# Patman86/SVT-AV1-Mod-by-Patman

Measured on AMD Instinct MI355X. Metric: encoded fps (4K 10-bit preset 8) + ME+txfm HBM GB/s vs roofline, 1/2/4/8 GPU, higher is better.
Workload: dtype u8 (ME) / int32 (transform)

## Files before the change

### include/svt_hip_txfm.h

```cpp
#ifndef SVT_HIP_TXFM_H
#define SVT_HIP_TXFM_H

#include "svt_hip.h"

#ifdef __cplusplus
extern "C" {
#endif

#define SVT_HIP_FWD_DECL(W, H)                                                                                     \
    SVT_HIP_API void svt_av1_fwd_txfm2d_##W##x##H##_hip(int16_t *input, int32_t *output, uint32_t input_stride,    \
                                                        int32_t transform_type, uint8_t bit_depth);               \
    SVT_HIP_API void svt_av1_fwd_txfm2d_##W##x##H##_N2_hip(int16_t *input, int32_t *output, uint32_t input_stride, \
                                                           int32_t transform_type, uint8_t bit_depth);            \
    SVT_HIP_API void svt_av1_fwd_txfm2d_##W##x##H##_N4_hip(int16_t *input, int32_t *output, uint32_t input_stride, \
                                                           int32_t transform_type, uint8_t bit_depth);
SVT_HIP_FWD_DECL(4, 4) SVT_HIP_FWD_DECL(8, 8) SVT_HIP_FWD_DECL(16, 16) SVT_HIP_FWD_DECL(32, 32) SVT_HIP_FWD_DECL(64, 64)
SVT_HIP_FWD_DECL(4, 8) SVT_HIP_FWD_DECL(8, 4) SVT_HIP_FWD_DECL(8, 16) SVT_HIP_FWD_DECL(16, 8) SVT_HIP_FWD_DECL(16, 32)
SVT_HIP_FWD_DECL(32, 16) SVT_HIP_FWD_DECL(32, 64) SVT_HIP_FWD_DECL(64, 32) SVT_HIP_FWD_DECL(4, 16) SVT_HIP_FWD_DECL(16, 4)
SVT_HIP_FWD_DECL(8, 32) SVT_HIP_FWD_DECL(32, 8) SVT_HIP_FWD_DECL(16, 64) SVT_HIP_FWD_DECL(64, 16)

SVT_HIP_API uint64_t svt_handle_transform16x64_hip(int32_t *output);
SVT_HIP_API uint64_t svt_handle_transform32x64_hip(int32_t *output);
SVT_HIP_API uint64_t svt_handle_transform64x16_hip(int32_t *output);
SVT_HIP_API uint64_t svt_handle_transform64x32_hip(int32_t *output);
// ... 95 lines not shown
typedef struct SvtHipTxfmDesc {
    uint64_t residual_off;
    uint64_t coeff_off;
    uint64_t qcoeff_off, dqcoeff_off;
    uint64_t pred_off, recon_off;
    uint64_t iscan_off;
    uint64_t qm_off, iqm_off;
    uint32_t residual_stride;
    uint32_t pred_stride, recon_stride;
    int16_t  zbin[2], round[2], quant[2], quant_shift[2], dequant[2];
    uint8_t  tx_type, shape , bit_depth, quant_mode, log_scale, flags;
    uint8_t  dist_w, dist_h;
} SvtHipTxfmDesc;

typedef struct SvtHipTxfmResult {
    uint64_t three_quad_energy;
    uint16_t eob;
    uint16_t pad_;
    uint32_t satd;
} SvtHipTxfmResult;

SVT_HIP_API int32_t svt_hip_txfm_quant_batch(uint8_t *d_base, const SvtHipTxfmDesc *d_desc, SvtHipTxfmResult *d_result,
                                             uint32_t n_blocks, uint32_t w, uint32_t h, void *stream);

SVT_HIP_API int32_t svt_hip_txfm_distortion_batch(const uint8_t *d_base, const SvtHipTxfmDesc *d_desc, uint64_t (*d_distortion)[2],
                                                  uint32_t n_blocks, uint32_t w, uint32_t h, void *stream);

SVT_HIP_API int32_t svt_hip_quantize_batch(uint8_t *d_base, const SvtHipTxfmDesc *d_desc, SvtHipTxfmResult *d_result,
                                           uint32_t n_blocks, uint32_t n_coeffs, void *stream);

typedef struct SvtHipCoeffCost {
    int32_t txb_skip[13][2];
    int32_t base_eob[4][3];
    int32_t base[42][8];
    int32_t eob_extra[9][2];
    int32_t dc_sign[3][2];
    int32_t lps[21][26];
} SvtHipCoeffCost;

typedef struct SvtHipRateTables {
    SvtHipCoeffCost coeff[5][2];
    int32_t         eob[7][2][2][11];
    int32_t         intra_tx_type[3][4][13][17];
    int32_t         inter_tx_type[4][4][17];
} SvtHipRateTables;

// ... 164 lines not shown
```

### svt-av1-mod-by-patman_amd/csrc/common.hpp

```cpp
#pragma once

#include <hip/hip_runtime.h>
#include <stddef.h>
#include <stdint.h>
#include <string.h>

#include "../../include/svt_hip.h"
#include "../../include/svt_hip_me.h"

namespace svthip {

void set_error(const char *fmt, ...);

hipStream_t resolve_stream(void *stream);

struct Scratch {
    uint8_t *dev    = nullptr;
    uint8_t *pinned = nullptr;
    size_t   dev_cap = 0, pinned_cap = 0;
    uint8_t *device(size_t bytes);
    uint8_t *host(size_t bytes, size_t keep = 0);
};

bool ensure_init();
int  cu_count();
hipError_t ensure_event(hipEvent_t &ev);

struct GuardedBuf {
    uint8_t   *dev = nullptr, *pinned = nullptr;
    size_t     cap = 0;
    hipEvent_t ev  = nullptr;
    bool       pending = false;
    bool       held    = false;
    hipError_t acquire(size_t bytes, size_t grow_to, bool host_writes, hipStream_t st, const char **what);
    hipError_t release(hipStream_t st);
};

struct ThreadState {
    char       err[512] = "";
    bool       bound    = false;
    int        slot     = -1;
    GuardedBuf ring[4];
    int        ring_next = 0;
    Scratch    scratch;
    GuardedBuf wiener_aux;
    GuardedBuf txfm_perm;
    hipEvent_t produced = nullptr;
};
ThreadState &tls();

class TierBCall {
public:
    TierBCall(const char *fn, void *stream);
    ~TierBCall() { release(); }
    TierBCall(const TierBCall &)            = delete;
    TierBCall &operator=(const TierBCall &) = delete;
    bool        ok() const { return status_ == SVT_HIP_OK; }
    int32_t     status() const { return status_; }
    hipStream_t stream() const { return st_; }
    void       *stage(const void *host, size_t bytes);
    void       *take(GuardedBuf &b, size_t bytes, size_t grow_to);
    int32_t     finish();

private:
    void       *fail(hipError_t e, const char *what);
    bool        hold(GuardedBuf &b, size_t bytes, size_t grow_to, bool host_writes);
    void        release();
    const char *fn_;
    hipStream_t st_     = nullptr;
// ... 100 lines not shown
```

### svt-av1-mod-by-patman_amd/csrc/runtime.cpp

```cpp
#include <atomic>
#include <cstdarg>
#include <cstdio>
#include <cstdlib>
#include <cstring>
#include <mutex>

#include "common.hpp"

namespace svthip {

#ifndef SVT_HIP_STREAM_POOL
#define SVT_HIP_STREAM_POOL 8
#endif
namespace {
constexpr int STREAM_POOL = SVT_HIP_STREAM_POOL;
struct Process {
    std::atomic<int> device{-1};
    std::atomic<int> sticky{-1};
    std::atomic<int> cus{0};
    std::mutex       mutex;
    std::atomic<hipStream_t> pool[STREAM_POOL];
    std::mutex               pool_mutex;
    std::atomic<int>         next_thread{0};
};
// ... 122 lines not shown
}
bool TierBCall::hold(GuardedBuf &b, size_t bytes, size_t grow_to, bool host_writes) {
    if (!ok())
        return false;
    if (b.held)
        return fail(hipErrorInvalidValue, "buffer still held by an enclosing call") != nullptr;
    const char      *what;
    const hipError_t e = b.acquire(bytes, grow_to, host_writes, st_, &what);
    if (e != hipSuccess)
        return fail(e, what) != nullptr;
    b.held = true, held_[n_held_++] = &b;
    return true;
}
void *TierBCall::stage(const void *host, size_t bytes) {
    ThreadState &t = tls();
    GuardedBuf  &s = t.ring[t.ring_next];
    if (!hold(s, bytes, bytes < 65536 ? 65536 : bytes * 2, true))
        return nullptr;
    t.ring_next = (t.ring_next + 1) % 4;
    memcpy(s.pinned, host, bytes);
    const hipError_t e = hipMemcpyAsync(s.dev, s.pinned, bytes, hipMemcpyHostToDevice, st_);
    return e == hipSuccess ? s.dev : fail(e, "hipMemcpyAsync");
}
void *TierBCall::take(GuardedBuf &b, size_t bytes, size_t grow_to) { return hold(b, bytes, grow_to, false) ? b.dev : nullptr; }
void TierBCall::release() {
    for (int i = 0; i < n_held_; i++) {
        const hipError_t e = held_[i]->release(st_);
        if (e != hipSuccess)
            fail(e, "hipEventRecord");
        held_[i]->held = false;
    }
    n_held_ = 0;
}
int32_t TierBCall::finish() {
    const hipError_t e = ok() ? hipGetLastError() : hipSuccess;
    if (e != hipSuccess)
        fail(e, "launch");
    release();
    return status_;
}

namespace {
struct SavedSlot {
    char   name[96];
    void **slot;
    void  *cpu_fn;
};
// ... 352 lines not shown
```

### svt-av1-mod-by-patman_amd/csrc/txfm.hip

```cpp
#include <cmath>
#include <cstdio>
#include <cstdlib>
#include <cstring>
#include <mutex>

#include "../../include/svt_hip_txfm.h"
#include "common.hpp"
#include "txfm_block.hpp"

using namespace svthip;
using namespace svthip::txd;
using namespace svthip::txb;

namespace {

template <int W, int H>
__global__ __launch_bounds__((Geo<W, H>::NT * Geo<W, H>::L), (Geo<W, H>::MINW)) void txfm_kernel(uint8_t *__restrict__ base,
                                                                            const SvtHipTxfmDesc *__restrict__ descs,
                                                                            SvtHipTxfmResult *__restrict__ results,
                                                                            uint32_t n, const uint32_t *__restrict__ perm) {
    using G = Geo<W, H>;
    constexpr int L = G::L, PW = G::PW, NT = G::NT;
    __shared__ int32_t buf[NT][H * PW];
    const int          t = threadIdx.x % L, slot = threadIdx.x / L;
    const uint32_t     i    = blockIdx.x * NT + slot;
    const bool         live = i < n;
    const uint32_t     tb   = live ? (perm ? perm[i] : i) : 0;
    txfm_block<W, H>(base, descs[tb], results + tb, live, t, buf[slot]);
}

constexpr uint32_t GROUP_CHUNK = 4096, GROUP_MIN_BLOCKS = 2048;
__global__ __launch_bounds__(1024) void group_by_type_kernel(const SvtHipTxfmDesc *__restrict__ descs, uint32_t n, uint32_t *__restrict__ perm) {
    __shared__ uint32_t hist[16], start[16];
    const uint32_t base = blockIdx.x * GROUP_CHUNK;
    if (threadIdx.x < 16)
        hist[threadIdx.x] = 0;
    __syncthreads();
    uint32_t key[GROUP_CHUNK / 1024], rank[GROUP_CHUNK / 1024];
#pragma unroll
    for (uint32_t k = 0; k < GROUP_CHUNK / 1024; k++) {
        const uint32_t i = base + k * 1024 + threadIdx.x;
        key[k] = i < n ? (descs[i].tx_type & 15u) : 16u;
        if (key[k] < 16)
            rank[k] = atomicAdd(&hist[key[k]], 1u);
    }
    __syncthreads();
// ... 82 lines not shown
std::once_flag g_tables_once;
int32_t        g_tables_rc = SVT_HIP_OK;
void           upload_tables() {
    constexpr CosTable tab = make_cospi();
    for (int b = 0; b < 4; b++)
        for (int j = 0; j < 64; j++)
            if (tab.v[b][j] != (int32_t)llround(cos(M_PI * j / 128.0) * (double)(1 << (10 + b)))) {
                set_error("transform constant table self-check failed");
                g_tables_rc = SVT_HIP_ERR_RUNTIME;
            }
}
}

int32_t svthip::txfm_ready() {
    if (!ensure_init())
        return SVT_HIP_ERR_NO_DEVICE;
    std::call_once(g_tables_once, upload_tables);
    return g_tables_rc;
}

namespace {

template <int W, int H>
void launch_txfm(uint8_t *base, const SvtHipTxfmDesc *descs, SvtHipTxfmResult *res, uint32_t n, hipStream_t st) {
    using G = Geo<W, H>;
    const uint32_t *perm = nullptr;
    static const bool group = getenv("SVTAV1_HIP_GROUP_TX") != nullptr;
    if (G::NT > 1 && n >= GROUP_MIN_BLOCKS && group && st) {
        TierBCall c("transform grouping", (void *)st);
        perm = (const uint32_t *)c.take(tls().txfm_perm, (size_t)n * sizeof(uint32_t), (size_t)n * sizeof(uint32_t));
        if (perm)
            hipLaunchKernelGGL(group_by_type_kernel, dim3((n + GROUP_CHUNK - 1) / GROUP_CHUNK), dim3(1024), 0, st, descs, n, (uint32_t *)perm);
        hipLaunchKernelGGL((txfm_kernel<W, H>), dim3((n + G::NT - 1) / G::NT), dim3(G::NT * G::L), 0, st, base, descs, res, n, perm);
        return;
    }
    hipLaunchKernelGGL((txfm_kernel<W, H>), dim3((n + G::NT - 1) / G::NT), dim3(G::NT * G::L), 0, st, base, descs, res, n, perm);
}

bool dispatch_txfm(uint32_t w, uint32_t h, uint8_t *base, const SvtHipTxfmDesc *descs, SvtHipTxfmResult *res, uint32_t n,
                   hipStream_t st) {
#define CASE(W, H)                                \
    if (w == W && h == H) {                       \
        launch_txfm<W, H>(base, descs, res, n, st); \
        return true;                              \
    }
    CASE(4, 4) CASE(8, 8) CASE(16, 16) CASE(32, 32) CASE(64, 64) CASE(4, 8) CASE(8, 4) CASE(8, 16) CASE(16, 8) CASE(16, 32)
    CASE(32, 16) CASE(32, 64) CASE(64, 32) CASE(4, 16) CASE(16, 4) CASE(8, 32) CASE(32, 8) CASE(16, 64) CASE(64, 16)
#undef CASE
    return false;
}

}

extern "C" int32_t svt_hip_txfm_quant_batch(uint8_t *d_base, const SvtHipTxfmDesc *d_desc, SvtHipTxfmResult *d_result,
                                            uint32_t n_blocks, uint32_t w, uint32_t h, void *stream) {
    if (!d_base || !d_desc || !d_result) {
        set_error("svt_hip_txfm_quant_batch: NULL pointer");
        return SVT_HIP_ERR_BAD_PARAMETER;
    }
    const int32_t rc = txfm_ready();
    if (rc != SVT_HIP_OK)
        return rc;
    if (n_blocks == 0)
        return SVT_HIP_OK;
    if (!dispatch_txfm(w, h, d_base, d_desc, d_result, n_blocks, resolve_stream(stream))) {
        set_error("svt_hip_txfm_quant_batch: %ux%u is not an AV1 transform size", w, h);
        return SVT_HIP_ERR_BAD_PARAMETER;
    }
    SVT_HIP_CHECK(hipGetLastError());
    return SVT_HIP_OK;
}

extern "C" int32_t svt_hip_quantize_batch(uint8_t *d_base, const SvtHipTxfmDesc *d_desc, SvtHipTxfmResult *d_result,
                                          uint32_t n_blocks, uint32_t n_coeffs, void *stream) {
    if (!d_base || !d_desc || !d_result || n_coeffs == 0) {
        set_error("svt_hip_quantize_batch: bad argument");
        return SVT_HIP_ERR_BAD_PARAMETER;
    }
    const int32_t rc = txfm_ready();
    if (rc != SVT_HIP_OK)
        return rc;
    if (n_blocks == 0)
        return SVT_HIP_OK;
    hipLaunchKernelGGL(quantize_kernel, dim3(n_blocks), dim3(256), 0, resolve_stream(stream), d_base, d_desc, d_result, n_coeffs);
    SVT_HIP_CHECK(hipGetLastError());
    return SVT_HIP_OK;
}

namespace {


struct OneBlock : TierAStage {
    size_t off_desc, off_res;
    OneBlock(const char *what) : TierAStage(what, txfm_ready() == SVT_HIP_OK), off_desc(in(nullptr, 256)), off_res(out(256)) {
        memset(desc(), 0, sizeof(SvtHipTxfmDesc));
    }
    SvtHipTxfmDesc         *desc() const { return host<SvtHipTxfmDesc>(off_desc); }
    const SvtHipTxfmResult *result() const { return host<SvtHipTxfmResult>(off_res); }
    void run(int w, int h) {
        upload();
        if (!dispatch_txfm((uint32_t)w, (uint32_t)h, dev(0), dev<const SvtHipTxfmDesc>(off_desc), dev<SvtHipTxfmResult>(off_res), 1, stream()))
            fatal("bad transform size");
    }
};

void fwd_tier_a(int w, int h, int shape, int16_t *input, int32_t *output, uint32_t stride, int32_t tx_type, uint8_t bd) {
    OneBlock     a("forward transform");
    const size_t out_bytes = (size_t)w * h * 4;
    const size_t off_in = a.in(input, ((size_t)(h - 1) * stride + w) * 2, 16), off_out = a.out(out_bytes + 16);
    SvtHipTxfmDesc *dsc = a.desc();
    dsc->residual_off = off_in, dsc->coeff_off = off_out;
    dsc->qcoeff_off = dsc->dqcoeff_off = dsc->qm_off = dsc->iqm_off = dsc->iscan_off = dsc->pred_off = dsc->recon_off = SVT_HIP_NO_OFFSET;
    dsc->residual_stride = stride;
    dsc->tx_type = (uint8_t)tx_type, dsc->shape = (uint8_t)shape, dsc->bit_depth = bd;
    dsc->quant_mode = SVT_HIP_QUANT_NONE, dsc->flags = SVT_HIP_TX_FWD | SVT_HIP_TX_FULLCOEFF;
    a.run(w, h);
    a.finish(off_out, out_bytes);
    memcpy(output, a.host(off_out), out_bytes);
}

template <class PIX>
void inv_tier_a(int w, int h, const int32_t *input, const PIX *out_r, int32_t stride_r, PIX *out_w, int32_t stride_w, int32_t tx_type,
                int32_t bd) {
    OneBlock     a("inverse transform");
// ... 113 lines not shown
```

### svt-av1-mod-by-patman_amd/csrc/txfm_block.hpp

```cpp
#pragma once
#include <cstdint>

#include "../../include/svt_hip_txfm.h"
#include "common.hpp"
#include "txfm_device.hpp"

namespace svthip {
int32_t txfm_ready();
namespace txb {
using namespace svthip::txd;


constexpr int8_t FWD_SHIFT[5][5][3] = {
    {{2, 0, 0}, {2, -1, 0}, {2, -1, 0}, {0, 0, 0}, {0, 0, 0}},   {{2, -1, 0}, {2, -1, 0}, {2, -2, 0}, {2, -2, 0}, {0, 0, 0}},
    {{2, -1, 0}, {2, -2, 0}, {2, -2, 0}, {2, -4, 0}, {0, -2, 0}}, {{0, 0, 0}, {2, -2, 0}, {2, -4, 0}, {2, -4, 0}, {0, -2, -2}},
    {{0, 0, 0}, {0, 0, 0}, {2, -4, 0}, {2, -4, -2}, {0, -2, -2}}};
constexpr int8_t FWD_COS_COL[5][5] = {{13, 13, 13, 0, 0}, {13, 13, 13, 12, 0}, {13, 13, 13, 12, 13}, {0, 13, 13, 12, 13}, {0, 0, 13, 12, 13}};
constexpr int8_t FWD_COS_ROW[5][5] = {{13, 13, 12, 0, 0}, {13, 13, 13, 12, 0}, {13, 13, 12, 13, 12}, {0, 12, 13, 12, 11}, {0, 0, 12, 11, 10}};
constexpr int8_t INV_SHIFT0[5][5]  = {{0, 0, -1, 0, 0}, {0, -1, -1, -2, 0}, {-1, -1, -2, -1, -2}, {0, -2, -1, -2, -1}, {0, 0, -2, -1, -2}};
__device__ const uint8_t VTX_D[16] = {0, 1, 0, 1, 2, 0, 2, 1, 2, 3, 0, 3, 1, 3, 2, 3};
__device__ const uint8_t HTX_D[16] = {0, 0, 1, 1, 0, 2, 2, 2, 1, 3, 3, 0, 3, 1, 3, 2};

constexpr int cmax(int a, int b) { return a > b ? a : b; }
constexpr int cmin(int a, int b) { return a < b ? a : b; }
constexpr int pow2floor(int v) {
    int p = 1;
    while (p * 2 <= v) p *= 2;
    return p;
}
#ifndef SVT_HIP_TX64_WAVES
#define SVT_HIP_TX64_WAVES 1
#endif
template <int W, int H>
struct Geo {
    static constexpr int L  = cmax(W, H);
    static constexpr int PW = W + 1;
    static constexpr int NT = cmax(1, 64 / L);
    static constexpr int IW = cmin(W, 32), IH = cmin(H, 32);
    static constexpr int MINW = L == 32 ? 3 : (L == 8 ? 8 : (L == 64 ? SVT_HIP_TX64_WAVES : 1));
    static constexpr int WI = clog2(W) - 2, HI = clog2(H) - 2;
    static constexpr bool RECT = (W == 2 * H) || (H == 2 * W);
};

struct QP {
    int32_t        zbin[2], round[2], quant[2], qshift[2], dequant[2];
    int32_t        log_scale, mode;
    const uint8_t *qm, *iqm;
    bool           simple;
};
__device__ __forceinline__ int32_t rpot(int32_t v, int n) { return (v + ((1 << n) >> 1)) >> n; }
__device__ __forceinline__ void load_qp(QP &q, const SvtHipTxfmDesc &d, const uint8_t *base) {
    q.log_scale = d.log_scale, q.mode = d.quant_mode;
    bool small = true;
    for (int i = 0; i < 2; i++) {
        q.zbin[i]    = rpot(d.zbin[i], d.log_scale);
        q.round[i]   = rpot(d.round[i], d.log_scale);
        q.quant[i]   = d.quant[i];
        q.qshift[i]  = d.quant_shift[i];
        q.dequant[i] = d.dequant[i];
        small = small && q.zbin[i] >= 0 && q.zbin[i] < 65536 && q.round[i] >= 0 && q.round[i] < 32768 && q.quant[i] >= -32768 && q.quant[i] < 32768 &&
            q.qshift[i] >= 0 && q.qshift[i] < 65536 && q.dequant[i] >= 0 && q.dequant[i] < 32768;
    }
// ... 130 lines not shown
};

template <int IW, int IH, int L, int PW>
__device__ __forceinline__ void coop_store_tile(const int32_t *__restrict__ lds, int32_t *__restrict__ g, int t) {
    constexpr int NCH = IW * IH / 4;
    if ((((uintptr_t)g) & 15) == 0) {
#pragma unroll
        for (int k = 0; k < (NCH + L - 1) / L; k++) {
            const int q = k * L + t;
            if (q < NCH) {
                const int e = 4 * q, r = e / IW, c = e % IW;
                int4      v;
                v.x = lds[r * PW + c], v.y = lds[r * PW + c + 1], v.z = lds[r * PW + c + 2], v.w = lds[r * PW + c + 3];
                typedef int v4i __attribute__((ext_vector_type(4)));
                const v4i nv = {v.x, v.y, v.z, v.w};
                __builtin_nontemporal_store(nv, (v4i *)g + q);
            }
        }
    } else {
        for (int e = t; e < IW * IH; e += L) g[e] = lds[(e / IW) * PW + e % IW];
    }
}

template <int W, int H, bool BLKERR = false>
__device__ __forceinline__ void txfm_block(uint8_t *__restrict__ base, const SvtHipTxfmDesc &d, SvtHipTxfmResult *__restrict__ result,
                                           const bool live, const int t, int32_t *__restrict__ lds) {
    static_assert(!BLKERR || (W != 64 && H != 64), "three_quad_energy is the 64-point energy for those sizes");
    using G = Geo<W, H>;
    constexpr int L = G::L, PW = G::PW, IW = G::IW, IH = G::IH;
    const int vk = VTX_D[d.tx_type & 15], hk = HTX_D[d.tx_type & 15];
    const bool ud = vk == 2, lr = hk == 2;
    const int  bd = d.bit_depth;
    const int  bdi = bd == 8 ? 0 : (bd == 10 ? 1 : (bd == 12 ? 2 : -1));
    const bool do_fwd = d.flags & SVT_HIP_TX_FWD, do_inv = d.flags & SVT_HIP_TX_INV;
    constexpr int sh0 = FWD_SHIFT[G::WI][G::HI][0], sh1 = FWD_SHIFT[G::WI][G::HI][1], sh2 = FWD_SHIFT[G::WI][G::HI][2];
    int32_t  row[W];
#pragma unroll
    for (int c = 0; c < W; c++) row[c] = 0;

    if (do_fwd) {
        if (live && t < W) {
            int32_t        v[H];
            {
                const ptrdiff_t step = ud ? -(ptrdiff_t)d.residual_stride : (ptrdiff_t)d.residual_stride;
                const ptrdiff_t row0 = (ud ? (ptrdiff_t)(H - 1) * d.residual_stride : 0) + t;
                if (!(d.flags & SVT_HIP_TX_SRC_PRED)) {
                    const int16_t *rp = (const int16_t *)(base + d.residual_off) + row0;
#pragma unroll
                    for (int r = 0; r < H; r++, rp += step) v[r] = (int32_t)((uint32_t)(int32_t)__builtin_nontemporal_load(rp) << sh0);
                } else {
                    const ptrdiff_t pstep = ud ? -(ptrdiff_t)d.pred_stride : (ptrdiff_t)d.pred_stride;
                    const ptrdiff_t prow0 = (ud ? (ptrdiff_t)(H - 1) * d.pred_stride : 0) + t;
                    if (d.flags & SVT_HIP_TX_PIXEL16) {
                        const uint16_t *sp = (const uint16_t *)(base + d.residual_off) + row0;
                        const uint16_t *pp = (const uint16_t *)(base + d.pred_off) + prow0;
#pragma unroll
                        for (int r = 0; r < H; r++, sp += step, pp += pstep)
                            v[r] = (int32_t)((uint32_t)(int32_t)(int16_t)(*sp - *pp) << sh0);
                    } else {
                        const uint8_t *sp = base + d.residual_off + row0, *pp = base + d.pred_off + prow0;
#pragma unroll
                        for (int r = 0; r < H; r++, sp += step, pp += pstep) v[r] = (int32_t)((uint32_t)((int32_t)*sp - (int32_t)*pp) << sh0);
                    }
                }
            }
            if (__all(max_abs<H>(v) <= (uint32_t)FWD_FAST_LIMIT[G::HI][kind_index(vk)][FWD_COS_COL[G::WI][G::HI] - 10])) {
                fwd1d<Fast, H>(v, vk, FWD_COS_COL[G::WI][G::HI]);
                if constexpr (sh1 < 0) {
#pragma unroll
                    for (int r = 0; r < H; r++) v[r] = Fast::rs(v[r], -sh1);
                }
            } else {
                fwd1d<Exact, H>(v, vk, FWD_COS_COL[G::WI][G::HI]);
                if constexpr (sh1 < 0) {
#pragma unroll
                    for (int r = 0; r < H; r++) v[r] = rshift64(v[r], -sh1);
                }
            }
            const int cc = lr ? W - 1 - t : t;
#pragma unroll
            for (int r = 0; r < H; r++) lds[r * PW + cc] = v[r];
        }
        __syncthreads();
        if (live && t < H) {
#pragma unroll
            for (int c = 0; c < W; c++) row[c] = lds[t * PW + c];
            if (__all(max_abs<W>(row) <= (uint32_t)FWD_FAST_LIMIT[G::WI][kind_index(hk)][FWD_COS_ROW[G::WI][G::HI] - 10])) {
                fwd1d<Fast, W>(row, hk, FWD_COS_ROW[G::WI][G::HI]);
                if constexpr (sh2 < 0) {
#pragma unroll
                    for (int c = 0; c < W; c++) row[c] = Fast::rs(row[c], -sh2);
                }
            } else {
                fwd1d<Exact, W>(row, hk, FWD_COS_ROW[G::WI][G::HI]);
                if constexpr (sh2 < 0) {
#pragma unroll
                    for (int c = 0; c < W; c++) row[c] = rshift64(row[c], -sh2);
                }
            }
            const int kw = W >> d.shape, kh = H >> d.shape;
#pragma unroll
            for (int c = 0; c < W; c++) {
                int32_t x = row[c];
                if (G::RECT)
                    x = rshift64((int64_t)x * 5793, 12);
                row[c] = (t < kh && c < kw) ? x : 0;
            }
        }
    }
    uint64_t energy = 0;
    if constexpr (W == 64 || H == 64) {
        if (do_fwd && live && t < H) {
#pragma unroll
            for (int c = 0; c < W; c++)
                if (t >= IH || c >= IW)
                    energy += (uint64_t)((int64_t)row[c] * (int64_t)row[c]);
        }
        energy = group_sum64<L>(energy);
    }
    uint32_t satd = 0;
    if (do_fwd && (d.flags & SVT_HIP_TX_SATD)) {
        if (live && t < IH) {
#pragma unroll
            for (int c = 0; c < IW; c++) satd += (uint32_t)(row[c] < 0 ? -row[c] : row[c]);
        }
        satd = group_sum32<L>(satd);
    }
    uint32_t eob = 0;
    uint32_t iscv[(IW + 1) / 2];
    {
        const bool      qon = live && t < IH && d.quant_mode != SVT_HIP_QUANT_NONE;
        const uint16_t *isp = (const uint16_t *)(base + (qon ? d.iscan_off : 0)) + (qon ? t * IW : 0);
#pragma unroll
        for (int c = 0; c < IW; c += 2) iscv[c / 2] = qon ? ((uint32_t)isp[c] | ((uint32_t)isp[c + 1] << 16)) : 0u;
    }
    if (live && do_fwd && d.coeff_off != SVT_HIP_NO_OFFSET && (d.flags & SVT_HIP_TX_FULLCOEFF) && t < H) {
        int32_t *co = (int32_t *)(base + d.coeff_off) + t * W;
#pragma unroll
        for (int c = 0; c < W; c++) co[c] = row[c];
    }
    if (live && t < IH) {
        if (do_fwd && d.coeff_off != SVT_HIP_NO_OFFSET && !(d.flags & SVT_HIP_TX_FULLCOEFF)) {
            int32_t *co = (int32_t *)(base + d.coeff_off) + t * IW;
#pragma unroll
            for (int c = 0; c < IW; c++) co[c] = row[c];
        }
        if (d.quant_mode != SVT_HIP_QUANT_NONE) {
            QP q;
            load_qp(q, d, base);
            if (!do_fwd) {
                const int32_t *ci = (const int32_t *)(base + d.coeff_off) + t * IW;
#pragma unroll
                for (int c = 0; c < IW; c++) row[c] = ci[c];
            }
            const bool btype = q.mode == SVT_HIP_QUANT_B || q.mode == SVT_HIP_QUANT_B_HBD;
            const int  path  = (q.simple && max_abs<IW>(row) <= 32767u) ? (btype ? 1 : 2) : 0;
            const bool all1 = __all(path == 1), all2 = __all(path == 2);
#pragma unroll
            for (int c = 0; c < IW; c++) {
                const uint32_t rc = (uint32_t)(t * IW + c);
                const int      ac = (c > 0) | (t > 0);
                int32_t        qc, dqc;
                if (all1)
                    quant_small<true>(q, row[c], ac, qc, dqc);
                else if (all2)
                    quant_small<false>(q, row[c], ac, qc, dqc);
                else
                    quant_one(q, row[c], rc, qc, dqc);
                const uint32_t pos = qc ? ((iscv[c / 2] >> (16 * (c & 1))) & 0xffffu) + 1u : 0u;
                eob                = pos > eob ? pos : eob;
                lds[t * PW + c] = qc;
                if constexpr (BLKERR) {
                    const int64_t e = (int64_t)row[c] - (int64_t)dqc;
                    energy += (uint64_t)(e * e);
                }
                row[c]          = dqc;
            }
        } else if (do_inv && !do_fwd) {
            const int32_t *dqi = (const int32_t *)(base + d.dqcoeff_off) + t * IW;
#pragma unroll
            for (int c = 0; c < IW; c++) row[c] = dqi[c];
        }
    }
    eob = group_max<L>(eob);
    if constexpr (BLKERR)
        energy = group_sum64<L>(energy);
    {
        const bool quant = live && d.quant_mode != SVT_HIP_QUANT_NONE;
        __syncthreads();
        if (quant && d.qcoeff_off != SVT_HIP_NO_OFFSET)
            coop_store_tile<IW, IH, L, PW>(lds, (int32_t *)(base + d.qcoeff_off), t);
        __syncthreads();
        if (quant && t < IH) {
#pragma unroll
            for (int c = 0; c < IW; c++) lds[t * PW + c] = row[c];
        }
        __syncthreads();
        if (quant && d.dqcoeff_off != SVT_HIP_NO_OFFSET)
            coop_store_tile<IW, IH, L, PW>(lds, (int32_t *)(base + d.dqcoeff_off), t);
    }
    if (live && t == 0) {
        SvtHipTxfmResult r;
        r.three_quad_energy = energy;
        r.eob               = (uint16_t)eob;
        r.pad_ = 0, r.satd = satd;
        *result = r;
    }
    __syncthreads();
    if (live && do_inv && t < H) {
        const int range_row = bd == 8 ? 16 : (bd == 10 ? 18 : 20);
        const int clamp_in  = bd + 8;
        bool      any       = false;
#pragma unroll
        for (int c = 0; c < W; c++) {
            int32_t x = (t < IH && c < IW) ? row[c] : 0;
            if (G::RECT)
                x = rshift64((int64_t)x * 2896, 12);
            row[c] = clampv<true>(x, clamp_in);
            any |= row[c] != 0;
        }
        if (any) {
            constexpr int ish0 = INV_SHIFT0[G::WI][G::HI];
            if (__all(bdi >= 0 && INV_FAST_OK[bdi < 0 ? 0 : bdi][0][G::WI][kind_index(hk)] != 0)) {
                inv1d<Fast, W>(row, hk, range_row);
                if constexpr (ish0 < 0) {
#pragma unroll
                    for (int c = 0; c < W; c++) row[c] = Fast::rs(row[c], -ish0);
                }
            } else {
                inv1d<Exact, W>(row, hk, range_row);
                if constexpr (ish0 < 0) {
#pragma unroll
                    for (int c = 0; c < W; c++) row[c] = rshift64(row[c], -ish0);
                }
            }
        }
#pragma unroll
        for (int c = 0; c < W; c++) lds[t * PW + c] = row[c];
    }
    __syncthreads();
    if (live && do_inv && t < W) {
        int32_t   v[H];
        const int range_col = bd == 12 ? 18 : 16, col_clamp = bd + 6 > 16 ? bd + 6 : 16;
        const int cc = lr ? W - 1 - t : t;
#pragma unroll
        for (int r = 0; r < H; r++) v[r] = r < IH ? clampv<true>(lds[r * PW + cc], col_clamp) : 0;
        if (__all(bdi >= 0 && INV_FAST_OK[bdi < 0 ? 0 : bdi][1][G::HI][kind_index(vk)] != 0)) {
            inv1d<Fast, H>(v, vk, range_col);
#pragma unroll
            for (int r = 0; r < H; r++) v[r] = Fast::rs(v[r], 4);
        } else {
            inv1d<Exact, H>(v, vk, range_col);
#pragma unroll
            for (int r = 0; r < H; r++) v[r] = rshift64(v[r], 4);
        }
        const ptrdiff_t r0 = ud ? H - 1 : 0, rs = ud ? -(ptrdiff_t)d.recon_stride : (ptrdiff_t)d.recon_stride;
        uint32_t predv[(H + 1) / 2];
        {
            const ptrdiff_t ps = ud ? -(ptrdiff_t)d.pred_stride : (ptrdiff_t)d.pred_stride;
            if (d.flags & SVT_HIP_TX_PIXEL16) {
                const uint16_t *pr = (const uint16_t *)(base + d.pred_off) + r0 * (ptrdiff_t)d.pred_stride + t;
#pragma unroll
                for (int r = 0; r < H; r += 2) predv[r / 2] = (uint32_t)__builtin_nontemporal_load(pr + (ptrdiff_t)r * ps) | ((uint32_t)__builtin_nontemporal_load(pr + (ptrdiff_t)(r + 1) * ps) << 16);
            } else {
                const uint8_t *pr = base + d.pred_off + r0 * (ptrdiff_t)d.pred_stride + t;
#pragma unroll
                for (int r = 0; r < H; r += 2) predv[r / 2] = (uint32_t)pr[(ptrdiff_t)r * ps] | ((uint32_t)pr[(ptrdiff_t)(r + 1) * ps] << 16);
            }
        }
        const PixelClip clip((d.flags & SVT_HIP_TX_PIXEL16) ? bd : 8);
        if (d.flags & SVT_HIP_TX_PIXEL16) {
            uint16_t *rc = (uint16_t *)(base + d.recon_off) + r0 * (ptrdiff_t)d.recon_stride + t;
#pragma unroll
            for (int r = 0; r < H; r++, rc += rs) __builtin_nontemporal_store(clip.add((uint16_t)(predv[r / 2] >> (16 * (r & 1))), v[r]), rc);
        } else {
            uint8_t *rc = base + d.recon_off + r0 * (ptrdiff_t)d.recon_stride + t;
#pragma unroll
            for (int r = 0; r < H; r++, rc += rs) *rc = (uint8_t)clip.add((uint16_t)(predv[r / 2] >> (16 * (r & 1))), v[r]);
        }
    }
}

}
}
```

### svt-av1-mod-by-patman_amd/svtav1_hip/prototypes.py

```python
PROTOTYPES = {
    "svt_aom_cdef_find_dir_dual_hip": (None, ("c_void_p", "c_void_p", "c_int", "c_void_p", "c_void_p", "c_int32", "c_void_p", "c_void_p")),
    "svt_aom_cdef_find_dir_hip": ("c_uint8", ("c_void_p", "c_int32", "c_void_p", "c_int32")),
    "svt_aom_copy_rect8_8bit_to_16bit_hip": (None, ("c_void_p", "c_int32", "c_void_p", "c_int32", "c_int32", "c_int32")),
    "svt_aom_downsample_2d_hip": (None, ("c_void_p", "c_uint32", "c_uint32", "c_uint32", "c_void_p", "c_uint32", "c_uint32")),
    "svt_aom_highbd_lpf_horizontal_14_hip": (None, ("c_void_p", "c_int32", "c_void_p", "c_void_p", "c_void_p", "c_int32")),
    "svt_aom_highbd_lpf_horizontal_4_hip": (None, ("c_void_p", "c_int32", "c_void_p", "c_void_p", "c_void_p", "c_int32")),
    "svt_aom_highbd_lpf_horizontal_6_hip": (None, ("c_void_p", "c_int32", "c_void_p", "c_void_p", "c_void_p", "c_int32")),
    "svt_aom_highbd_lpf_horizontal_8_hip": (None, ("c_void_p", "c_int32", "c_void_p", "c_void_p", "c_void_p", "c_int32")),
    "svt_aom_highbd_lpf_vertical_14_hip": (None, ("c_void_p", "c_int32", "c_void_p", "c_void_p", "c_void_p", "c_int32")),
    "svt_aom_highbd_lpf_vertical_4_hip": (None, ("c_void_p", "c_int32", "c_void_p", "c_void_p", "c_void_p", "c_int32")),
    "svt_aom_highbd_lpf_vertical_6_hip": (None, ("c_void_p", "c_int32", "c_void_p", "c_void_p", "c_void_p", "c_int32")),
    "svt_aom_highbd_lpf_vertical_8_hip": (None, ("c_void_p", "c_int32", "c_void_p", "c_void_p", "c_void_p", "c_int32")),
    "svt_aom_highbd_quantize_b_hip": (None, ("c_void_p", "c_ssize_t", "c_void_p", "c_void_p", "c_void_p", "c_void_p", "c_void_p", "c_void_p", "c_void_p", "c_void_p", "c_void_p", "c_void_p", "c_void_p", "c_void_p", "c_int32")),
    "svt_aom_highbd_subtract_block_hip": (None, ("c_int", "c_int", "c_void_p", "c_ssize_t", "c_void_p", "c_ssize_t", "c_void_p", "c_ssize_t", "c_int")),
    "svt_aom_lpf_horizontal_14_hip": (None, ("c_void_p", "c_int32", "c_void_p", "c_void_p", "c_void_p")),
    "svt_aom_lpf_horizontal_4_hip": (None, ("c_void_p", "c_int32", "c_void_p", "c_void_p", "c_void_p")),
    "svt_aom_lpf_horizontal_6_hip": (None, ("c_void_p", "c_int32", "c_void_p", "c_void_p", "c_void_p")),
    "svt_aom_lpf_horizontal_8_hip": (None, ("c_void_p", "c_int32", "c_void_p", "c_void_p", "c_void_p")),
    "svt_aom_lpf_vertical_14_hip": (None, ("c_void_p", "c_int32", "c_void_p", "c_void_p", "c_void_p")),
    "svt_aom_lpf_vertical_4_hip": (None, ("c_void_p", "c_int32", "c_void_p", "c_void_p", "c_void_p")),
    "svt_aom_lpf_vertical_6_hip": (None, ("c_void_p", "c_int32", "c_void_p", "c_void_p", "c_void_p")),
    "svt_aom_lpf_vertical_8_hip": (None, ("c_void_p", "c_int32", "c_void_p", "c_void_p", "c_void_p")),
    "svt_aom_quantize_b_hip": (None, ("c_void_p", "c_ssize_t", "c_void_p", "c_void_p", "c_void_p", "c_void_p", "c_void_p", "c_void_p", "c_void_p", "c_void_p", "c_void_p", "c_void_p", "c_void_p", "c_void_p", "c_int32")),
    "svt_aom_sad_16b_kernel_hip": ("c_uint32", ("c_void_p", "c_uint32", "c_void_p", "c_uint32", "c_uint32", "c_uint32")),
# ... 133 lines not shown
    "svt_handle_transform64x16_hip": ("c_uint64", ("c_void_p",)),
    "svt_handle_transform64x32_N2_N4_hip": ("c_uint64", ("c_void_p",)),
    "svt_handle_transform64x32_hip": ("c_uint64", ("c_void_p",)),
    "svt_handle_transform64x64_N2_N4_hip": ("c_uint64", ("c_void_p",)),
    "svt_handle_transform64x64_hip": ("c_uint64", ("c_void_p",)),
    "svt_hip_analysis_frames": ("c_int32", ("c_void_p", "c_uint32", "c_int32", "c_int32", "c_void_p")),
    "svt_hip_blend_batch": ("c_int32", ("c_void_p", "c_uint32", "c_void_p")),
    "svt_hip_cdef_apply_frame": ("c_int32", ("c_void_p", "c_uint32", "c_void_p", "c_void_p", "c_int32", "c_int32", "c_void_p", "c_void_p", "c_void_p")),
    "svt_hip_cdef_apply_plane": ("c_int32", ("c_void_p", "c_void_p", "c_void_p", "c_int32", "c_int32", "c_void_p", "c_void_p", "c_void_p")),
    "svt_hip_cdef_pick_strengths": ("c_int32", ("c_void_p", "c_void_p", "c_void_p", "c_void_p", "c_void_p", "c_void_p", "c_void_p", "c_uint64", "c_void_p")),
    "svt_hip_cdef_pick_workspace_bytes": ("c_uint64", ("c_uint32", "c_int32")),
    "svt_hip_cdef_search_plane": ("c_int32", ("c_void_p", "c_void_p", "c_void_p", "c_void_p", "c_void_p", "c_void_p", "c_void_p")),
    "svt_hip_cfl_predict_batch": ("c_int32", ("c_void_p", "c_uint32", "c_void_p")),
    "svt_hip_comm_create": ("c_int32", ("c_void_p", "c_int32", "c_int32", "c_void_p")),
    "svt_hip_comm_destroy": ("c_int32", ("c_void_p",)),
    "svt_hip_comm_get_unique_id": ("c_int32", ("c_void_p",)),
    "svt_hip_compound_mask_search_batch": ("c_int32", ("c_void_p", "c_void_p", "c_uint32", "c_void_p")),
    "svt_hip_compute_units": ("c_int32", ()),
    "svt_hip_convolve_batch": ("c_int32", ("c_void_p", "c_uint32", "c_void_p")),
    "svt_hip_convolve_sr_batch": ("c_int32", ("c_void_p", "c_uint32", "c_void_p")),
    "svt_hip_copy": ("c_int32", ("c_void_p", "c_void_p", "c_size_t", "c_void_p")),
    "svt_hip_debug_inject_failure": (None, ("c_int32",)),
    "svt_hip_debug_tier_a_broken": ("c_int32", ("c_int32",)),
    "svt_hip_device_count": ("c_int32", ()),
    "svt_hip_download": ("c_int32", ("c_void_p", "c_void_p", "c_size_t", "c_void_p")),
    "svt_hip_download_2d": ("c_int32", ("c_void_p", "c_size_t", "c_void_p", "c_size_t", "c_size_t", "c_size_t", "c_void_p")),
    "svt_hip_event_destroy": ("c_int32", ("c_void_p",)),
    "svt_hip_free": ("c_int32", ("c_void_p",)),
    "svt_hip_gm_refine": ("c_int32", ("c_void_p", "c_void_p", "c_void_p", "c_int32", "c_int64", "c_void_p", "c_void_p")),
    "svt_hip_host_alloc": ("c_int32", ("c_void_p", "c_size_t")),
    "svt_hip_host_free": ("c_int32", ("c_void_p",)),
    "svt_hip_init": ("c_int32", ("c_int32",)),
    "svt_hip_install_rtcd": ("c_int32", ("c_void_p", "c_uint32", "c_void_p")),
    "svt_hip_install_rtcd_me": ("c_int32", ("c_void_p", "c_uint32")),
    "svt_hip_intra_predict_batch": ("c_int32", ("c_void_p", "c_uint32", "c_void_p")),
    "svt_hip_intra_predict_batch_packed": ("c_int32", ("c_void_p", "c_uint32", "c_uint32", "c_void_p")),
    "svt_hip_intra_search_frames": ("c_int32", ("c_void_p", "c_uint32", "c_void_p")),
    "svt_hip_last_error": ("c_char_p", ()),
    "svt_hip_loop_filter_frame": ("c_int32", ("c_void_p", "c_void_p")),
    "svt_hip_malloc": ("c_int32", ("c_void_p", "c_size_t")),
    "svt_hip_me_b64_count": ("c_uint32", ("c_uint32", "c_uint32")),
    "svt_hip_me_frames": ("c_int32", ("c_void_p", "c_uint32", "c_void_p")),
    "svt_hip_me_frames_dev": ("c_int32", ("c_void_p", "c_uint32", "c_uint32", "c_void_p")),
    "svt_hip_me_validate_jobs": ("c_int32", ("c_void_p", "c_uint32", "c_void_p")),
    "svt_hip_memset": ("c_int32", ("c_void_p", "c_int", "c_size_t", "c_void_p")),
    "svt_hip_pad_plane": ("c_int32", ("c_void_p", "c_void_p")),
# ... 65 lines not shown
```

Measured before the change: 5852.

## Add lean specialized transform kernel with device-side fallback list to general kernel

New measurement: 5980 (median of 6 runs). 1.02x the previous value.

```diff
diff --git a/include/svt_hip_txfm.h b/include/svt_hip_txfm.h
--- a/include/svt_hip_txfm.h
+++ b/include/svt_hip_txfm.h
@@ -141,6 +141,7 @@
 
 SVT_HIP_API int32_t svt_hip_txfm_quant_batch(uint8_t *d_base, const SvtHipTxfmDesc *d_desc, SvtHipTxfmResult *d_result,
                                              uint32_t n_blocks, uint32_t w, uint32_t h, void *stream);
+SVT_HIP_API int32_t svt_hip_debug_txfm_fallback_blocks(uint32_t *out);
 
 SVT_HIP_API int32_t svt_hip_txfm_distortion_batch(const uint8_t *d_base, const SvtHipTxfmDesc *d_desc, uint64_t (*d_distortion)[2],
                                                   uint32_t n_blocks, uint32_t w, uint32_t h, void *stream);
diff --git a/svt-av1-mod-by-patman_amd/csrc/common.hpp b/svt-av1-mod-by-patman_amd/csrc/common.hpp
--- a/svt-av1-mod-by-patman_amd/csrc/common.hpp
+++ b/svt-av1-mod-by-patman_amd/csrc/common.hpp
@@ -45,6 +45,8 @@
     Scratch    scratch;
     GuardedBuf wiener_aux;
     GuardedBuf txfm_perm;
+    hipStream_t     txfm_fast_stream = nullptr;
+    const uint32_t *txfm_fast_hdr    = nullptr;
     hipEvent_t produced = nullptr;
 };
 ThreadState &tls();
diff --git a/svt-av1-mod-by-patman_amd/csrc/runtime.cpp b/svt-av1-mod-by-patman_amd/csrc/runtime.cpp
--- a/svt-av1-mod-by-patman_amd/csrc/runtime.cpp
+++ b/svt-av1-mod-by-patman_amd/csrc/runtime.cpp
@@ -168,7 +168,12 @@
     const hipError_t e = hipMemcpyAsync(s.dev, s.pinned, bytes, hipMemcpyHostToDevice, st_);
     return e == hipSuccess ? s.dev : fail(e, "hipMemcpyAsync");
 }
-void *TierBCall::take(GuardedBuf &b, size_t bytes, size_t grow_to) { return hold(b, bytes, grow_to, false) ? b.dev : nullptr; }
+void *TierBCall::take(GuardedBuf &b, size_t bytes, size_t grow_to) {
+    ThreadState &t = tls();
+    if (&b == &t.txfm_perm)
+        t.txfm_fast_stream = nullptr, t.txfm_fast_hdr = nullptr;
+    return hold(b, bytes, grow_to, false) ? b.dev : nullptr;
+}
 void TierBCall::release() {
     for (int i = 0; i < n_held_; i++) {
         const hipError_t e = held_[i]->release(st_);
diff --git a/svt-av1-mod-by-patman_amd/csrc/txfm.hip b/svt-av1-mod-by-patman_amd/csrc/txfm.hip
--- a/svt-av1-mod-by-patman_amd/csrc/txfm.hip
+++ b/svt-av1-mod-by-patman_amd/csrc/txfm.hip
@@ -14,14 +14,51 @@
 
 namespace {
 
+enum : uint32_t { FB_COUNT = 0, FB_LIST = 16 };
+
 template <int W, int H>
-__global__ __launch_bounds__((Geo<W, H>::NT * Geo<W, H>::L), (Geo<W, H>::MINW)) void txfm_kernel(uint8_t *__restrict__ base,
+__global__ __launch_bounds__((Geo<W, H>::NT * Geo<W, H>::L), (Geo<W, H>::LEANW)) void txfm_kernel(uint8_t *__restrict__ base,
                                                                             const SvtHipTxfmDesc *__restrict__ descs,
                                                                             SvtHipTxfmResult *__restrict__ results,
-                                                                            uint32_t n, const uint32_t *__restrict__ perm) {
+                                                                            uint32_t n, const uint32_t *__restrict__ perm,
+                                                                            uint32_t *__restrict__ fb) {
+    using G = Geo<W, H>;
+    constexpr int L = G::L, PW = G::PW, NT = G::NT;
+    static_assert(NT * L == 64, "one wave per workgroup: a bail-out is uniform over the workgroup");
+    __shared__ int32_t buf[NT][H * PW];
+    const int          t = threadIdx.x % L, slot = threadIdx.x / L;
+    const uint32_t     i    = blockIdx.x * NT + slot;
+    const bool         live = i < n;
+    const uint32_t     tb   = live ? (perm ? perm[i] : i) : 0;
+    if constexpr (!G::LEAN) {
+        txfm_block<W, H>(base, descs[tb], results + tb, live, t, buf[slot]);
+    } else {
+        if (txfm_block<W, H, false, true>(base, descs[tb], results + tb, live, t, buf[slot]))
+            return;
+        const uint32_t left = n - blockIdx.x * NT, n_live = left < (uint32_t)NT ? left : (uint32_t)NT;
+        uint32_t       at   = 0;
+        if (threadIdx.x == 0)
+            at = atomicAdd(&fb[FB_COUNT], n_live);
+        at = (uint32_t)__shfl((int)at, 0, 64);
+        if (live && t == 0)
+            fb[FB_LIST + at + slot] = tb;
+    }
+}
+
+template <int W, int H>
+__global__ __launch_bounds__((Geo<W, H>::NT * Geo<W, H>::L), (Geo<W, H>::MINW)) void txfm_general_kernel(uint8_t *__restrict__ base,
+                                                                            const SvtHipTxfmDesc *__restrict__ descs,
+                                                                            SvtHipTxfmResult *__restrict__ results,
+                                                                            uint32_t n, const uint32_t *__restrict__ perm,
+                                                                            const uint32_t *__restrict__ count) {
     using G = Geo<W, H>;
     constexpr int L = G::L, PW = G::PW, NT = G::NT;
     __shared__ int32_t buf[NT][H * PW];
+    if (count) {
+        n = *count;
+        if (blockIdx.x * NT >= n)
+            return;
+    }
     const int          t = threadIdx.x % L, slot = threadIdx.x / L;
     const uint32_t     i    = blockIdx.x * NT + slot;
     const bool         live = i < n;
@@ -150,26 +187,48 @@
 namespace {
 
 template <int W, int H>
-void launch_txfm(uint8_t *base, const SvtHipTxfmDesc *descs, SvtHipTxfmResult *res, uint32_t n, hipStream_t st) {
+void launch_txfm(uint8_t *base, const SvtHipTxfmDesc *descs, SvtHipTxfmResult *res, uint32_t n, hipStream_t st, bool batch) {
     using G = Geo<W, H>;
     const uint32_t *perm = nullptr;
+    const dim3      grid((n + G::NT - 1) / G::NT), wg(G::NT * G::L);
+    ThreadState    &ts = tls();
+    auto            launch_general = [&](const uint32_t *pm) {
+        if constexpr (G::LEAN)
+            hipLaunchKernelGGL((txfm_general_kernel<W, H>), grid, wg, 0, st, base, descs, res, n, pm, (const uint32_t *)nullptr);
+        else
+            hipLaunchKernelGGL((txfm_kernel<W, H>), grid, wg, 0, st, base, descs, res, n, pm, (uint32_t *)nullptr);
+    };
+    ts.txfm_fast_stream = nullptr;
     static const bool group = getenv("SVTAV1_HIP_GROUP_TX") != nullptr;
-    if (G::NT > 1 && n >= GROUP_MIN_BLOCKS && group && st) {
-        TierBCall c("transform grouping", (void *)st);
-        perm = (const uint32_t *)c.take(tls().txfm_perm, (size_t)n * sizeof(uint32_t), (size_t)n * sizeof(uint32_t));
-        if (perm)
+    static const bool fast_on = !(getenv("SVTAV1_HIP_TXFM_FAST") && atoi(getenv("SVTAV1_HIP_TXFM_FAST")) == 0);
+    const bool fast = G::LEAN && fast_on && batch, grouped = G::NT > 1 && n >= GROUP_MIN_BLOCKS && group;
+    if ((fast || grouped) && st) {
+        TierBCall    c("transform scratch", (void *)st);
+        const size_t bytes = ((size_t)FB_LIST + (size_t)n * (grouped ? 2 : 1)) * sizeof(uint32_t);
+        uint32_t    *fb    = (uint32_t *)c.take(ts.txfm_perm, bytes, bytes);
+        if (fb && grouped) {
+            perm = fb + FB_LIST + n;
             hipLaunchKernelGGL(group_by_type_kernel, dim3((n + GROUP_CHUNK - 1) / GROUP_CHUNK), dim3(1024), 0, st, descs, n, (uint32_t *)perm);
-        hipLaunchKernelGGL((txfm_kernel<W, H>), dim3((n + G::NT - 1) / G::NT), dim3(G::NT * G::L), 0, st, base, descs, res, n, perm);
+        }
+        if constexpr (G::LEAN) {
+            if (fb && fast && hipMemsetAsync(fb + FB_COUNT, 0, sizeof(uint32_t), st) == hipSuccess) {
+                hipLaunchKernelGGL((txfm_kernel<W, H>), grid, wg, 0, st, base, descs, res, n, perm, fb);
+                hipLaunchKernelGGL((txfm_general_kernel<W, H>), grid, wg, 0, st, base, descs, res, n, fb + FB_LIST, fb + FB_COUNT);
+                ts.txfm_fast_stream = st, ts.txfm_fast_hdr = fb;
+                return;
+            }
+        }
+        launch_general(perm);
         return;
     }
-    hipLaunchKernelGGL((txfm_kernel<W, H>), dim3((n + G::NT - 1) / G::NT), dim3(G::NT * G::L), 0, st, base, descs, res, n, perm);
+    launch_general(perm);
 }
 
 bool dispatch_txfm(uint32_t w, uint32_t h, uint8_t *base, const SvtHipTxfmDesc *descs, SvtHipTxfmResult *res, uint32_t n,
-                   hipStream_t st) {
+                   hipStream_t st, bool batch) {
 #define CASE(W, H)                                \
     if (w == W && h == H) {                       \
-        launch_txfm<W, H>(base, descs, res, n, st); \
+        launch_txfm<W, H>(base, descs, res, n, st, batch); \
         return true;                              \
     }
     CASE(4, 4) CASE(8, 8) CASE(16, 16) CASE(32, 32) CASE(64, 64) CASE(4, 8) CASE(8, 4) CASE(8, 16) CASE(16, 8) CASE(16, 32)
@@ -191,11 +250,25 @@
         return rc;
     if (n_blocks == 0)
         return SVT_HIP_OK;
-    if (!dispatch_txfm(w, h, d_base, d_desc, d_result, n_blocks, resolve_stream(stream))) {
+    if (!dispatch_txfm(w, h, d_base, d_desc, d_result, n_blocks, resolve_stream(stream), true)) {
         set_error("svt_hip_txfm_quant_batch: %ux%u is not an AV1 transform size", w, h);
         return SVT_HIP_ERR_BAD_PARAMETER;
     }
     SVT_HIP_CHECK(hipGetLastError());
+    return SVT_HIP_OK;
+}
+
+extern "C" int32_t svt_hip_debug_txfm_fallback_blocks(uint32_t *out) {
+    if (!out) {
+        set_error("svt_hip_debug_txfm_fallback_blocks: NULL pointer");
+        return SVT_HIP_ERR_BAD_PARAMETER;
+    }
+    *out = 0;
+    ThreadState &ts = tls();
+    if (!ts.txfm_fast_stream)
+        return SVT_HIP_OK;
+    SVT_HIP_CHECK(hipStreamSynchronize(ts.txfm_fast_stream));
+    SVT_HIP_CHECK(hipMemcpy(out, ts.txfm_fast_hdr + FB_COUNT, sizeof(uint32_t), hipMemcpyDeviceToHost));
     return SVT_HIP_OK;
 }
 
@@ -227,7 +300,7 @@
     const SvtHipTxfmResult *result() const { return host<SvtHipTxfmResult>(off_res); }
     void run(int w, int h) {
         upload();
-        if (!dispatch_txfm((uint32_t)w, (uint32_t)h, dev(0), dev<const SvtHipTxfmDesc>(off_desc), dev<SvtHipTxfmResult>(off_res), 1, stream()))
+        if (!dispatch_txfm((uint32_t)w, (uint32_t)h, dev(0), dev<const SvtHipTxfmDesc>(off_desc), dev<SvtHipTxfmResult>(off_res), 1, stream(), false))
             fatal("bad transform size");
     }
 };
diff --git a/svt-av1-mod-by-patman_amd/csrc/txfm_block.hpp b/svt-av1-mod-by-patman_amd/csrc/txfm_block.hpp
--- a/svt-av1-mod-by-patman_amd/csrc/txfm_block.hpp
+++ b/svt-av1-mod-by-patman_amd/csrc/txfm_block.hpp
@@ -38,6 +38,8 @@
     static constexpr int NT = cmax(1, 64 / L);
     static constexpr int IW = cmin(W, 32), IH = cmin(H, 32);
     static constexpr int MINW = L == 32 ? 3 : (L == 8 ? 8 : (L == 64 ? SVT_HIP_TX64_WAVES : 1));
+    static constexpr bool LEAN  = L == 16 || L == 32;
+    static constexpr int  LEANW = LEAN ? 1 : MINW;
     static constexpr int WI = clog2(W) - 2, HI = clog2(H) - 2;
     static constexpr bool RECT = (W == 2 * H) || (H == 2 * W);
 };
@@ -214,8 +216,19 @@
     }
 }
 
-template <int W, int H, bool BLKERR = false>
-__device__ __forceinline__ void txfm_block(uint8_t *__restrict__ base, const SvtHipTxfmDesc &d, SvtHipTxfmResult *__restrict__ result,
+template <int W, int H>
+__device__ __forceinline__ bool lean_class(const SvtHipTxfmDesc &d, const uint8_t *base) {
+    using G = Geo<W, H>;
+    const int vk = VTX_D[d.tx_type & 15], hk = HTX_D[d.tx_type & 15];
+    const int bdi = d.bit_depth == 8 ? 0 : (d.bit_depth == 10 ? 1 : -1);
+    QP q;
+    load_qp(q, d, base);
+    return (d.flags & ~(uint32_t)SVT_HIP_TX_PIXEL16) == (SVT_HIP_TX_FWD | SVT_HIP_TX_INV) && d.shape == 0 && d.coeff_off == SVT_HIP_NO_OFFSET &&
+        (q.mode == SVT_HIP_QUANT_B || q.mode == SVT_HIP_QUANT_B_HBD) && q.simple && bdi >= 0 &&
+        INV_FAST_OK[bdi < 0 ? 0 : bdi][0][G::WI][kind_index(hk)] != 0 && INV_FAST_OK[bdi < 0 ? 0 : bdi][1][G::HI][kind_index(vk)] != 0;
+}
+template <int W, int H, bool BLKERR = false, bool LEAN = false>
+__device__ __forceinline__ bool txfm_block(uint8_t *__restrict__ base, const SvtHipTxfmDesc &d, SvtHipTxfmResult *__restrict__ result,
                                            const bool live, const int t, int32_t *__restrict__ lds) {
     static_assert(!BLKERR || (W != 64 && H != 64), "three_quad_energy is the 64-point energy for those sizes");
     using G = Geo<W, H>;
@@ -224,7 +237,12 @@
     const bool ud = vk == 2, lr = hk == 2;
     const int  bd = d.bit_depth;
     const int  bdi = bd == 8 ? 0 : (bd == 10 ? 1 : (bd == 12 ? 2 : -1));
-    const bool do_fwd = d.flags & SVT_HIP_TX_FWD, do_inv = d.flags & SVT_HIP_TX_INV;
+    const bool do_fwd = LEAN || (d.flags & SVT_HIP_TX_FWD), do_inv = LEAN || (d.flags & SVT_HIP_TX_INV);
+    if constexpr (LEAN) {
+        if (!__all(!live || lean_class<W, H>(d, base)))
+            return false;
+    }
+    bool fast_ok = true;
     constexpr int sh0 = FWD_SHIFT[G::WI][G::HI][0], sh1 = FWD_SHIFT[G::WI][G::HI][1], sh2 = FWD_SHIFT[G::WI][G::HI][2];
     int32_t  row[W];
 #pragma unroll
@@ -236,7 +254,7 @@
             {
                 const ptrdiff_t step = ud ? -(ptrdiff_t)d.residual_stride : (ptrdiff_t)d.residual_stride;
                 const ptrdiff_t row0 = (ud ? (ptrdiff_t)(H - 1) * d.residual_stride : 0) + t;
-                if (!(d.flags & SVT_HIP_TX_SRC_PRED)) {
+                if (LEAN || !(d.flags & SVT_HIP_TX_SRC_PRED)) {
                     const int16_t *rp = (const int16_t *)(base + d.residual_off) + row0;
 #pragma unroll
                     for (int r = 0; r < H; r++, rp += step) v[r] = (int32_t)((uint32_t)(int32_t)__builtin_nontemporal_load(rp) << sh0);
@@ -262,6 +280,8 @@
 #pragma unroll
                     for (int r = 0; r < H; r++) v[r] = Fast::rs(v[r], -sh1);
                 }
+            } else if constexpr (LEAN) {
+                fast_ok = false;
             } else {
                 fwd1d<Exact, H>(v, vk, FWD_COS_COL[G::WI][G::HI]);
                 if constexpr (sh1 < 0) {
@@ -272,6 +292,10 @@
             const int cc = lr ? W - 1 - t : t;
 #pragma unroll
             for (int r = 0; r < H; r++) lds[r * PW + cc] = v[r];
+        }
+        if constexpr (LEAN) {
+            if (!__all(fast_ok))
+                return false;
         }
         __syncthreads();
         if (live && t < H) {
@@ -283,6 +307,8 @@
 #pragma unroll
                     for (int c = 0; c < W; c++) row[c] = Fast::rs(row[c], -sh2);
                 }
+            } else if constexpr (LEAN) {
+                fast_ok = false;
             } else {
                 fwd1d<Exact, W>(row, hk, FWD_COS_ROW[G::WI][G::HI]);
                 if constexpr (sh2 < 0) {
@@ -290,7 +316,7 @@
                     for (int c = 0; c < W; c++) row[c] = rshift64(row[c], -sh2);
                 }
             }
-            const int kw = W >> d.shape, kh = H >> d.shape;
+            const int kw = LEAN ? W : W >> d.shape, kh = LEAN ? H : H >> d.shape;
 #pragma unroll
             for (int c = 0; c < W; c++) {
                 int32_t x = row[c];
@@ -300,6 +326,10 @@
             }
         }
     }
+    if constexpr (LEAN) {
+        if (!__all(fast_ok && (!live || t >= IH || max_abs<IW>(row) <= 32767u)))
+            return false;
+    }
     uint64_t energy = 0;
     if constexpr (W == 64 || H == 64) {
         if (do_fwd && live && t < H) {
@@ -311,7 +341,7 @@
         energy = group_sum64<L>(energy);
     }
     uint32_t satd = 0;
-    if (do_fwd && (d.flags & SVT_HIP_TX_SATD)) {
+    if (!LEAN && do_fwd && (d.flags & SVT_HIP_TX_SATD)) {
         if (live && t < IH) {
 #pragma unroll
             for (int c = 0; c < IW; c++) satd += (uint32_t)(row[c] < 0 ? -row[c] : row[c]);
@@ -321,23 +351,23 @@
     uint32_t eob = 0;
     uint32_t iscv[(IW + 1) / 2];
     {
-        const bool      qon = live && t < IH && d.quant_mode != SVT_HIP_QUANT_NONE;
+        const bool      qon = live && t < IH && (LEAN || d.quant_mode != SVT_HIP_QUANT_NONE);
         const uint16_t *isp = (const uint16_t *)(base + (qon ? d.iscan_off : 0)) + (qon ? t * IW : 0);
 #pragma unroll
         for (int c = 0; c < IW; c += 2) iscv[c / 2] = qon ? ((uint32_t)isp[c] | ((uint32_t)isp[c + 1] << 16)) : 0u;
     }
-    if (live && do_fwd && d.coeff_off != SVT_HIP_NO_OFFSET && (d.flags & SVT_HIP_TX_FULLCOEFF) && t < H) {
+    if (!LEAN && live && do_fwd && d.coeff_off != SVT_HIP_NO_OFFSET && (d.flags & SVT_HIP_TX_FULLCOEFF) && t < H) {
         int32_t *co = (int32_t *)(base + d.coeff_off) + t * W;
 #pragma unroll
         for (int c = 0; c < W; c++) co[c] = row[c];
     }
     if (live && t < IH) {
-        if (do_fwd && d.coeff_off != SVT_HIP_NO_OFFSET && !(d.flags & SVT_HIP_TX_FULLCOEFF)) {
+        if (!LEAN && do_fwd && d.coeff_off != SVT_HIP_NO_OFFSET && !(d.flags & SVT_HIP_TX_FULLCOEFF)) {
             int32_t *co = (int32_t *)(base + d.coeff_off) + t * IW;
 #pragma unroll
             for (int c = 0; c < IW; c++) co[c] = row[c];
         }
-        if (d.quant_mode != SVT_HIP_QUANT_NONE) {
+        if (LEAN || d.quant_mode != SVT_HIP_QUANT_NONE) {
             QP q;
             load_qp(q, d, base);
             if (!do_fwd) {
@@ -346,8 +376,8 @@
                 for (int c = 0; c < IW; c++) row[c] = ci[c];
             }
             const bool btype = q.mode == SVT_HIP_QUANT_B || q.mode == SVT_HIP_QUANT_B_HBD;
-            const int  path  = (q.simple && max_abs<IW>(row) <= 32767u) ? (btype ? 1 : 2) : 0;
-            const bool all1 = __all(path == 1), all2 = __all(path == 2);
+            const int  path  = LEAN ? 1 : ((q.simple && max_abs<IW>(row) <= 32767u) ? (btype ? 1 : 2) : 0);
+            const bool all1 = LEAN || __all(path == 1), all2 = !LEAN && __all(path == 2);
 #pragma unroll
             for (int c = 0; c < IW; c++) {
                 const uint32_t rc = (uint32_t)(t * IW + c);
@@ -378,7 +408,7 @@
     if constexpr (BLKERR)
         energy = group_sum64<L>(energy);
     {
-        const bool quant = live && d.quant_mode != SVT_HIP_QUANT_NONE;
+        const bool quant = live && (LEAN || d.quant_mode != SVT_HIP_QUANT_NONE);
         __syncthreads();
         if (quant && d.qcoeff_off != SVT_HIP_NO_OFFSET)
             coop_store_tile<IW, IH, L, PW>(lds, (int32_t *)(base + d.qcoeff_off), t);
@@ -413,7 +443,7 @@
         }
         if (any) {
             constexpr int ish0 = INV_SHIFT0[G::WI][G::HI];
-            if (__all(bdi >= 0 && INV_FAST_OK[bdi < 0 ? 0 : bdi][0][G::WI][kind_index(hk)] != 0)) {
+            if (LEAN || __all(bdi >= 0 && INV_FAST_OK[bdi < 0 ? 0 : bdi][0][G::WI][kind_index(hk)] != 0)) {
                 inv1d<Fast, W>(row, hk, range_row);
                 if constexpr (ish0 < 0) {
 #pragma unroll
@@ -437,7 +467,7 @@
         const int cc = lr ? W - 1 - t : t;
 #pragma unroll
         for (int r = 0; r < H; r++) v[r] = r < IH ? clampv<true>(lds[r * PW + cc], col_clamp) : 0;
-        if (__all(bdi >= 0 && INV_FAST_OK[bdi < 0 ? 0 : bdi][1][G::HI][kind_index(vk)] != 0)) {
+        if (LEAN || __all(bdi >= 0 && INV_FAST_OK[bdi < 0 ? 0 : bdi][1][G::HI][kind_index(vk)] != 0)) {
             inv1d<Fast, H>(v, vk, range_col);
 #pragma unroll
             for (int r = 0; r < H; r++) v[r] = Fast::rs(v[r], 4);
@@ -471,7 +501,8 @@
             for (int r = 0; r < H; r++, rc += rs) *rc = (uint8_t)clip.add((uint16_t)(predv[r / 2] >> (16 * (r & 1))), v[r]);
         }
     }
-}
-
-}
-}
+    return true;
+}
+
+}
+}
diff --git a/svt-av1-mod-by-patman_amd/svtav1_hip/prototypes.py b/svt-av1-mod-by-patman_amd/svtav1_hip/prototypes.py
--- a/svt-av1-mod-by-patman_amd/svtav1_hip/prototypes.py
+++ b/svt-av1-mod-by-patman_amd/svtav1_hip/prototypes.py
@@ -179,6 +179,7 @@
     "svt_hip_copy": ("c_int32", ("c_void_p", "c_void_p", "c_size_t", "c_void_p")),
     "svt_hip_debug_inject_failure": (None, ("c_int32",)),
     "svt_hip_debug_tier_a_broken": ("c_int32", ("c_int32",)),
+    "svt_hip_debug_txfm_fallback_blocks": ("c_int32", ("c_void_p",)),
     "svt_hip_device_count": ("c_int32", ()),
     "svt_hip_download": ("c_int32", ("c_void_p", "c_void_p", "c_size_t", "c_void_p")),
     "svt_hip_download_2d": ("c_int32", ("c_void_p", "c_size_t", "c_void_p", "c_size_t", "c_size_t", "c_size_t", "c_void_p")),
```
